# liyi14/mx-DeepIM

Hardware: NVIDIA H100
Metric: 480x640 4-iter pose refinements/sec (higher is better)
Workload: dtype fp16

## Files before the change

mx-deepim_b200/csrc/conv_igemm.cuh:

```cuda
#pragma once
#include <cuda.h>
#include <cuda_fp16.h>
#include "common.cuh"
#include "wgmma.cuh"

namespace dim {

struct ConvKParams {
  CUtensorMap a_map[4];
  CUtensorMap a_lo_map[4];
  CUtensorMap b_map;
  CUtensorMap b_lo_map;
  CUtensorMap out_map[2];
  const __nv_bfloat16 *in_hi, *in_lo;
  int in_cols;
  int KH, KW, stride, cchunks;
  int BW, BH, n_col_tiles;
  int Hq, Ho, Wo, Bn;
  int out_Hp, out_Wp, out_py, out_px, Cout;
  int kblocks;
  float slope;
  const float *bias;
  __nv_bfloat16 *out_hi, *out_lo;
  int in_off_r, in_off_c;
// ... 117 lines not shown
  d |= (uint64_t)((lbo_bytes >> 4) & 0x3FFFu) << 16;
  d |= (uint64_t)((sbo_bytes >> 4) & 0x3FFFu) << 32;
  d |= (uint64_t)layout << 62;
  return d;
}
constexpr uint32_t kSW128 = 1u, kSW64 = 2u, kNoSwizzle = 0u;

__device__ __forceinline__ void regs_producer() { asm volatile("setmaxnreg.dec.sync.aligned.u32 40;"); }
__device__ __forceinline__ void regs_consumer() { asm volatile("setmaxnreg.inc.sync.aligned.u32 232;"); }

}

__device__ __forceinline__ uint32_t pack2_f16(float a, float b) {
  uint32_t r;
  asm("cvt.rn.satfinite.f16x2.f32 %0, %1, %2;" : "=r"(r) : "f"(b), "f"(a));
  return r;
}
__device__ __forceinline__ uint32_t pack2_bf16(float a, float b) {
  uint32_t r;
  asm("cvt.rn.bf16x2.f32 %0, %1, %2;" : "=r"(r) : "f"(b), "f"(a));
  return r;
}

constexpr int kConv1Slack = 2048;


__device__ __forceinline__ int frag_row(int t) { return ((t >> 5) << 4) + ((t & 31) >> 2); }

__device__ __forceinline__ uint32_t pack2_bf16_lo(float v0, float v1, uint32_t hi) {
  return pack2_bf16(v0 - __uint_as_float(hi << 16), v1 - __uint_as_float(hi & 0xFFFF0000u));
}

template <bool SPLIT3, bool F16>
__device__ __forceinline__ void epi_pack(float v0, float v1, float b0, float b1, float slope, uint32_t &hi, uint32_t &lo) {
  v0 += b0;
  v1 += b1;
  v0 = v0 > 0.f ? v0 : v0 * slope;
  v1 = v1 > 0.f ? v1 : v1 * slope;
  if (F16) {
    hi = pack2_f16(v0, v1);
  } else {
    hi = pack2_bf16(v0, v1);
    if (SPLIT3) lo = pack2_bf16_lo(v0, v1, hi);
  }
}

template <bool SPLIT3, bool F16>
__device__ __forceinline__ void store_pair(float v0, float v1, float2 b, float slope, __nv_bfloat16 *out_hi, __nv_bfloat16 *out_lo,
                                           long long off) {
  uint32_t h, l = 0;
  epi_pack<SPLIT3, F16>(v0, v1, b.x, b.y, slope, h, l);
  *reinterpret_cast<uint32_t *>(out_hi + off) = h;
  if (SPLIT3) *reinterpret_cast<uint32_t *>(out_lo + off) = l;
}

template <bool SPLIT3>
__device__ __forceinline__ void store_pair_generic(float v0, float v1, const ConvKParams &p, int n, bool valid, long long off,
                                                   long long add_off, long long mask_off) {
  if (!valid || n >= p.Cout) return;
  if (p.bias) {
    v0 += __ldg(p.bias + n);
    v1 += __ldg(p.bias + n + 1);
  }
  if (p.addend.p) {
    const __nv_bfloat162 a = *reinterpret_cast<const __nv_bfloat162 *>(p.addend.p + add_off);
    if (SPLIT3) {
      const __nv_bfloat162 al = *reinterpret_cast<const __nv_bfloat162 *>(p.addend.lo + add_off);
      v0 += __low2float(a) + __low2float(al);
      v1 += __high2float(a) + __high2float(al);
    } else {
      v0 += __low2float(a);
      v1 += __high2float(a);
    }
  }
  if (p.mask.p) {
    if (n < p.mask_climit) {
      const __nv_bfloat162 m = *reinterpret_cast<const __nv_bfloat162 *>(p.mask.p + mask_off);
      if (!(__low2float(m) > 0.f)) v0 *= p.slope;
      if (!(__high2float(m) > 0.f)) v1 *= p.slope;
    }
  } else {
    v0 = v0 > 0.f ? v0 : v0 * p.slope;
    v1 = v1 > 0.f ? v1 : v1 * p.slope;
  }
  if (SPLIT3) {
    const uint32_t h = pack2_bf16(v0, v1);
    *reinterpret_cast<uint32_t *>(p.out_hi + off) = h;
    *reinterpret_cast<uint32_t *>(p.out_lo + off) = pack2_bf16_lo(v0, v1, h);
  } else {
    *reinterpret_cast<__nv_bfloat162 *>(p.out_hi + off) = __floats2bfloat162_rn(v0, v1);
  }
}

template <int BLOCK_N, int STAGES, bool SPLIT3, int EPI>
struct ConvSmem2 {
  static constexpr int A_BYTES = 128 * 64 * 2;
  static constexpr int B_BYTES = BLOCK_N * 64 * 2;
  static constexpr int NPREC = SPLIT3 ? 2 : 1;
  static constexpr int STAGE_BYTES = (A_BYTES + B_BYTES) * NPREC;
  static constexpr int RING_BYTES = STAGES * STAGE_BYTES;
  static constexpr int LIMIT = 227 * 1024, FIXED = 1024  + 256 ;
  static constexpr bool TMA_EPI = EPI == 0 && !SPLIT3;
  static constexpr int STG_GROUPS =
      !TMA_EPI ? 0 : (RING_BYTES + 2 * BLOCK_N * 128 + FIXED <= LIMIT ? BLOCK_N / 64 : BLOCK_N / 128);
  static constexpr int STG_ROUNDS = TMA_EPI ? BLOCK_N / 64 / STG_GROUPS : 0;
  static constexpr int STG_BYTES = STG_GROUPS * 8192;
// ... 230 lines not shown
  const int g_lo = ck * rows_per_chunk;
  const int g_hi = min(rows_total, g_lo + rows_per_chunk);
  const int n_rows = max(0, g_hi - g_lo);
  const int n_strips = n_rows > 0 ? n_rows + 3 : 0;
  const int ow0 = ct * N;

  if (threadIdx.x == 0) {
    for (int s = 0; s < STAGES; ++s) {
      ptx::mbar_init(&full_bar[s], 1);
      ptx::mbar_init(&empty_bar[s], 2);
    }
    ptx::mbar_init(res_bar, 1);
    ptx::fence_barrier_init();
    ptx::prefetch_tmap(&p.b_map);
    ptx::prefetch_tmap(&p.out_map[0]);
  }
  __syncthreads();

  if (wgi == 0) {
    ptx::regs_producer();
    if (warp == 0 && n_rows > 0) {
      if (ptx::elect_one()) {
        ptx::mbar_expect_tx_raw(res_bar, (uint32_t)S::RES_BYTES);
        for (int kb = 0; kb < 16; ++kb) {
          ptx::tma_load_2d_raw(res + kb * S::TAP_BYTES, &p.b_map, res_bar, kb * 32, 0);
          if (SPLIT3) ptx::tma_load_2d_raw(res + (16 + kb) * S::TAP_BYTES, &p.b_lo_map, res_bar, kb * 32, 0);
        }
      }
      __syncwarp();
      const size_t plane = (size_t)p.in_cols * 16;
      const uint8_t *src_hi = reinterpret_cast<const uint8_t *>(p.in_hi) + (size_t)ow0 * 16;
      const uint8_t *src_lo = reinterpret_cast<const uint8_t *>(p.in_lo) + (size_t)ow0 * 16;
      for (int s = 0; s < n_strips; ++s) {
        const int slot = s % STAGES;
        ptx::mbar_wait(&empty_bar[slot], (((uint32_t)(s / STAGES)) & 1u) ^ 1u);
        uint8_t *st = ring + slot * S::STAGE_BYTES;
        if (g_lo + s >= rows_total) {
          if (ptx::elect_one()) ptx::mbar_arrive(&full_bar[slot]);
        } else if (ptx::elect_one()) {
          ptx::mbar_expect_tx_raw(&full_bar[slot], (uint32_t)(4 * S::PLANE_BYTES * S::NPREC));
          const size_t row = (size_t)(g_lo + s) * 4 * plane;
#pragma unroll
          for (int c = 0; c < 4; ++c) {
            ptx::bulk_load_raw(st + c * S::PLANE_BYTES, src_hi + row + c * plane, S::PLANE_BYTES, &full_bar[slot]);
            if (SPLIT3)
              ptx::bulk_load_raw(st + S::STRIP_BYTES + c * S::PLANE_BYTES, src_lo + row + c * plane, S::PLANE_BYTES, &full_bar[slot]);
          }
        }
        __syncwarp();
      }
    }
  } else if (n_rows > 0) {
    ptx::regs_consumer();
    const int set = wgi - 1, t = threadIdx.x & 127, lane = t & 31;
    const bool leader = t == 0;
    const int co = frag_row(t);
    const float b0 = __ldg(p.bias + co), b1 = __ldg(p.bias + co + 8);
    const uint32_t ring_a = ptx::smem_u32(ring);
    const uint64_t dring = ptx::gmma_desc(ring_a, S::PLANE_BYTES, 128, ptx::kNoSwizzle);
    const uint64_t dring3 = ptx::gmma_desc(ring_a, 2u * S::PLANE_BYTES, 128, ptx::kNoSwizzle) + 3u;
    const uint64_t lo_step = (uint64_t)(S::STRIP_BYTES >> 4);
    const uint64_t slot_step = (uint64_t)(S::STAGE_BYTES >> 4);
    const uint64_t kstep = (uint64_t)(2 * S::PLANE_BYTES >> 4);
    const uint64_t dres = ptx::gmma_desc(ptx::smem_u32(res), 16, 512, ptx::kSW64);
    const uint64_t dres_lo = dres + (uint64_t)((16 * S::TAP_BYTES) >> 4);
    uint8_t *my_stg = stg + set * S::NPREC * S::STG_BYTES;
    const int st_px = ((lane >> 4) << 3) + (lane & 7), st_chunk = 2 * (t >> 5) + ((lane >> 3) & 1);
    const uint32_t st_addr = ptx::smem_u32(my_stg) + (uint32_t)(st_px * 128 + ((st_chunk ^ (lane & 7)) << 4));
    ptx::mbar_wait(res_bar, 0);
    if (set == 1 && leader) ptx::mbar_arrive(&empty_bar[0]);
    for (int row = set; row < n_rows; row += 2) {
      float acc[N / 2];
#pragma unroll
      for (int dh = 0; dh < 4; ++dh) {
        const int s = row + dh;
        ptx::mbar_wait(&full_bar[s % STAGES], ((uint32_t)(s / STAGES)) & 1u);
      }
      wg::fence_acc(acc);
      wg::fence();
#pragma unroll
      for (int dh = 0; dh < 4; ++dh) {
        const uint64_t so = (uint64_t)((row + dh) % STAGES) * slot_step;
#pragma unroll
        for (int k = 0; k < 2; ++k) {
#pragma unroll
          for (int dw = 0; dw < 4; ++dw) {
            if ((dh == 3 || dw == 3) && k == 1) continue;
            const uint64_t db = (dw == 3 ? dring3 : dring + (uint64_t)dw + (uint64_t)k * kstep) + so;
            const uint64_t wo = (uint64_t)((dh * 4 + dw) * (S::TAP_BYTES >> 4) + 2 * k);
            wg::mma<N, F16, 0, 0>(acc, dres + wo, db, (dh | dw | k) ? 1u : 0u);
            if (SPLIT3) {
              wg::mma<N, false, 0, 0>(acc, dres + wo, db + lo_step, 1u);
              wg::mma<N, false, 0, 0>(acc, dres_lo + wo, db, 1u);
            }
          }
        }
      }
      wg::commit();
      wg::wait<0>();
      wg::fence_acc(acc);
      if (leader) {
        ptx::mbar_arrive(&empty_bar[row % STAGES]);
        ptx::mbar_arrive(&empty_bar[(row + 1) % STAGES]);
      }
      const int g = g_lo + row;
      const int n_img = g / p.Hq, oh = g - n_img * p.Hq;
      if (n_img < p.Bn && oh < p.Ho) {
        if (leader) ptx::bulk_wait_read0();
        ptx::named_bar_sync(1 + set, 128);
#pragma unroll
        for (int i = 0; i < N / 16; ++i) {
          uint32_t h[4], l[4] = {0, 0, 0, 0};
          epi_pack<SPLIT3, F16>(acc[8 * i + 0], acc[8 * i + 1], b0, b0, p.slope, h[0], l[0]);
          epi_pack<SPLIT3, F16>(acc[8 * i + 2], acc[8 * i + 3], b1, b1, p.slope, h[1], l[1]);
          epi_pack<SPLIT3, F16>(acc[8 * i + 4], acc[8 * i + 5], b0, b0, p.slope, h[2], l[2]);
          epi_pack<SPLIT3, F16>(acc[8 * i + 6], acc[8 * i + 7], b1, b1, p.slope, h[3], l[3]);
          ptx::stmatrix_x4_trans(st_addr + (uint32_t)(i * 16 * 128), h);
          if (SPLIT3) ptx::stmatrix_x4_trans(st_addr + (uint32_t)(S::STG_BYTES + i * 16 * 128), l);
        }
        ptx::fence_proxy_async();
        ptx::named_bar_sync(1 + set, 128);
        if (leader) {
#pragma unroll
          for (int q = 0; q < N / kConv1StoreN; ++q) {
            ptx::tma_store_4d(&p.out_map[0], my_stg + q * kConv1StoreN * 128, 0, ow0 + q * kConv1StoreN, oh, n_img);
            if (SPLIT3)
              ptx::tma_store_4d(&p.out_map[1], my_stg + S::STG_BYTES + q * kConv1StoreN * 128, 0, ow0 + q * kConv1StoreN, oh, n_img);
          }
          ptx::bulk_commit();
        }
      }
    }
    if (leader) ptx::bulk_wait0();
  }
}

template <int STAGES, bool SPLIT3, bool F16, int NB>
__global__ void __launch_bounds__(384, 1) conv1_rgbd_kernel(const __grid_constant__ ConvKParams p, const int rows_total,
                                                            const int rows_per_chunk, const int chunks_per_col,
                                                            const int strip_bytes ) {
  constexpr int NPREC = SPLIT3 ? 2 : 1;
  constexpr int TAP_BYTES = NB * 128, RES_BYTES = 16 * TAP_BYTES * NPREC;
  extern __shared__ uint8_t smem_raw[];
  uint8_t *smem = reinterpret_cast<uint8_t *>((reinterpret_cast<uintptr_t>(smem_raw) + 1023) & ~(uintptr_t)1023);
  uint8_t *res = smem;
  uint8_t *ring = smem + RES_BYTES;
  const int stage_bytes = strip_bytes * NPREC;
  uint64_t *full_bar = reinterpret_cast<uint64_t *>(ring + STAGES * stage_bytes + kConv1Slack);
  uint64_t *empty_bar = full_bar + STAGES;
  uint64_t *res_bar = empty_bar + STAGES;

  const int wgi = threadIdx.x >> 7, warp = threadIdx.x >> 5;
  const int R = p.BW + 3;
  const uint32_t LBO = (uint32_t)R * 16u;
  const int per_split = p.n_col_tiles * chunks_per_col;
  const int nsplit = blockIdx.x / per_split, cidx = blockIdx.x - nsplit * per_split;
  const int ct = cidx / chunks_per_col, ck = cidx - ct * chunks_per_col;
  const int n0 = nsplit * NB;
  const int g_lo = ck * rows_per_chunk;
  const int g_hi = min(rows_total, g_lo + rows_per_chunk);
  const int n_rows = max(0, g_hi - g_lo);
  const int n_strips = n_rows > 0 ? n_rows + 3 : 0;
  const int ow0 = ct * p.BW;

  if (threadIdx.x == 0) {
    for (int s = 0; s < STAGES; ++s) {
      ptx::mbar_init(&full_bar[s], 1);
      ptx::mbar_init(&empty_bar[s], 2);
    }
    ptx::mbar_init(res_bar, 1);
    ptx::fence_barrier_init();
    ptx::prefetch_tmap(&p.b_map);
    ptx::prefetch_tmap(&p.a_map[0]);
  }
  __syncthreads();

  if (wgi == 0) {
    ptx::regs_producer();
    if (warp == 0 && n_rows > 0) {
      if (ptx::elect_one()) {
// ... 99 lines not shown
```

mx-deepim_b200/csrc/net.cu:

```cuda
#include <cuda_fp16.h>
#include <string.h>

#include <memory>
#include <mutex>

#include "launch.cuh"
#include "net_state.cuh"

namespace dim {

static void build_geometry(NetState *ns, int H, int W) {
  int h = H, w = W;
  for (int i = 0; i < 10; ++i) {
    const LayerSpec &s = kLayers[i];
    LayerGeom &g = ns->g[i];
    g.Cin = s.Cin; g.Cout = s.Cout; g.k = s.k; g.stride = s.stride; g.pad = s.pad;
    g.Hin = h; g.Win = w;
    g.Ho = (h + 2 * s.pad - s.k) / s.stride + 1;
    g.Wo = (w + 2 * s.pad - s.k) / s.stride + 1;
    if (g.Ho < 1) g.Ho = 1;
    if (g.Wo < 1) g.Wo = 1;
    int Hp = h + 2 * s.pad, Wp = w + 2 * s.pad;
    if (s.stride == 2) { Hp += Hp & 1; Wp += Wp & 1; }
    g.py = g.px = s.pad;
    if (i == 0 && ns->input_depth) {
      g.Cin = 10;
      g.rows = Hp / 2; g.cols = Wp / 2; g.Cbuf = 64;
      g.KH = g.KW = 4; g.stride_eff = 1; g.Ceff = 64; g.Hq = g.rows;
      g.BLOCK_K = 64; g.BLOCK_N = 64;
    } else if (i == 0) {
      g.rows = Hp / 2; g.cols = Wp / 2; g.Cbuf = 32;
      g.KH = g.KW = 4; g.stride_eff = 1; g.Ceff = 32; g.Hq = g.rows;
      g.BLOCK_K = 32; g.BLOCK_N = 64;
    } else {
      g.rows = Hp; g.cols = Wp; g.Cbuf = s.Cin;
      g.KH = g.KW = s.k; g.stride_eff = s.stride; g.Ceff = s.Cin;
      g.Hq = (s.stride == 2) ? Hp / 2 : Hp;
      g.BLOCK_K = 64; g.BLOCK_N = s.Cout >= 256 ? 256 : 128;
    }
    int best_bw = 0, best_score = -1;
    for (int pass = 0; pass < 2 && best_bw == 0; ++pass)
      for (int d = 1; d <= g.Wo && d <= 128; ++d) {
        if (g.Wo % d) continue;
        if (pass == 0 && d < 8) continue;
        const int score = d * (128 / d) * 1000 + d;
        if (score > best_score) { best_score = score; best_bw = d; }
      }
    if (best_bw == 0) best_bw = 1;
    g.BW = best_bw; g.BH = 128 / best_bw;
    g.n_col_tiles = g.Wo > 0 ? g.Wo / g.BW : 0;
    if (i == 0) {
      const int nt = cdiv(g.Wo, 128);
      g.BW = cdiv(g.Wo, nt); g.BH = 1; g.n_col_tiles = nt;
    }
    g.kblocks = g.KH * g.KW * (g.Ceff / g.BLOCK_K);
    h = g.Ho; w = g.Wo;
  }
}

typedef CUresult (*EncodeTiledFn)(CUtensorMap *, CUtensorMapDataType, cuuint32_t, void *, const cuuint64_t *,
                                  const cuuint64_t *, const cuuint32_t *, const cuuint32_t *, CUtensorMapInterleave,
                                  CUtensorMapSwizzle, CUtensorMapL2promotion, CUtensorMapFloatOOBfill);
static EncodeTiledFn get_encode() {
  static EncodeTiledFn fn = nullptr;
  if (!fn) {
    void *p = nullptr;
    cudaDriverEntryPointQueryResult q;
    if (cudaGetDriverEntryPoint("cuTensorMapEncodeTiled", &p, cudaEnableDefault, &q) == cudaSuccess &&
        q == cudaDriverEntryPointSuccess)
      fn = reinterpret_cast<EncodeTiledFn>(p);
  }
  return fn;
}

int encode_map(CUtensorMap *m, void *base, int rank, const uint64_t *dims, const uint64_t *strides_bytes,
                      const uint32_t *box, int block_k ) {
  EncodeTiledFn fn = get_encode();
  DIM_REQUIRE(fn != nullptr, "cuTensorMapEncodeTiled entry point not available (driver too old?)");
  cuuint64_t gd[5]; cuuint64_t gs[5]; cuuint32_t bx[5]; cuuint32_t es[5];
  for (int i = 0; i < rank; ++i) { gd[i] = dims[i]; bx[i] = box[i]; es[i] = 1; }
  for (int i = 0; i < rank - 1; ++i) gs[i] = strides_bytes[i];
  CUresult r = fn(m, CU_TENSOR_MAP_DATA_TYPE_BFLOAT16, (cuuint32_t)rank, base, gd, gs, bx, es,
                  CU_TENSOR_MAP_INTERLEAVE_NONE,
                  block_k == 64 ? CU_TENSOR_MAP_SWIZZLE_128B
                                : (block_k == 32 ? CU_TENSOR_MAP_SWIZZLE_64B : CU_TENSOR_MAP_SWIZZLE_NONE),
                  CU_TENSOR_MAP_L2_PROMOTION_L2_256B, CU_TENSOR_MAP_FLOAT_OOB_FILL_NONE);
  if (r != CUDA_SUCCESS) {
    set_error("cuTensorMapEncodeTiled failed with CUresult %d (rank %d dims %llu %llu %llu box %u %u %u)", (int)r, rank,
              (unsigned long long)dims[0], (unsigned long long)dims[1], (unsigned long long)(rank > 2 ? dims[2] : 0),
              box[0], box[1], rank > 2 ? box[2] : 0);
    return 3;
  }
  return 0;
}

static int build_maps(NetState *ns, int B, bool f16, TensorMaps &tm) {
  for (int i = 0; i < 10; ++i) {
    const LayerGeom &g = ns->g[i];
    ConvKParams &kp = tm.kp[i];
    memset(&kp, 0, sizeof(kp));
    for (int lo = 0; lo < 2; ++lo) {
      __nv_bfloat16 *base = lo ? ns->act_lo[i] : ns->act_hi[i];
      CUtensorMap *maps = lo ? kp.a_lo_map : kp.a_map;
      const uint32_t box[3] = {(uint32_t)g.BLOCK_K, (uint32_t)g.BW, (uint32_t)(g.BH / 2)};
      if (i == 0 && ns->input_depth) {
        const uint64_t dims[4] = {8, (uint64_t)g.cols, 8, (uint64_t)B * g.rows};
        const uint64_t str[3] = {16, (uint64_t)g.cols * 16, (uint64_t)g.cols * 128};
        const uint32_t box4[4] = {8, (uint32_t)(g.BW + 3), 8, 1};
        if (int rc = encode_map(&maps[0], base, 4, dims, str, box4, 0)) return rc;
        maps[1] = maps[2] = maps[3] = maps[0];
      } else if (i == 0) {
      } else if (g.stride_eff == 1) {
        const uint64_t dims[3] = {(uint64_t)g.Cbuf, (uint64_t)g.cols, (uint64_t)B * g.rows};
        const uint64_t str[2] = {(uint64_t)g.Cbuf * 2, (uint64_t)g.cols * g.Cbuf * 2};
        if (int rc = encode_map(&maps[0], base, 3, dims, str, box, g.BLOCK_K)) return rc;
        maps[1] = maps[2] = maps[3] = maps[0];
      } else {
        for (int ph = 0; ph < 2; ++ph)
          for (int pw = 0; pw < 2; ++pw) {
            const uint64_t dims[3] = {(uint64_t)g.Cbuf, (uint64_t)g.cols / 2, (uint64_t)B * g.rows / 2};
            const uint64_t str[2] = {(uint64_t)2 * g.Cbuf * 2, (uint64_t)2 * g.cols * g.Cbuf * 2};
            __nv_bfloat16 *vb = base + ((size_t)ph * g.cols + pw) * g.Cbuf;
            if (int rc = encode_map(&maps[(ph << 1) | pw], vb, 3, dims, str, box, g.BLOCK_K)) return rc;
          }
      }
    }
    {
      const uint64_t Ktot = (uint64_t)g.KH * g.KW * g.Ceff;
      const uint64_t dims[2] = {Ktot, (uint64_t)g.Cout};
      const uint64_t str[1] = {Ktot * 2};
      const uint32_t box[2] = {(uint32_t)g.BLOCK_K, (uint32_t)(i == 0 && ns->input_depth ? 16 : g.BLOCK_N)};
      __nv_bfloat16 *wop = f16 ? ns->w_f16[i] : ns->w_hi[i];
      if (int rc = encode_map(&kp.b_map, wop, 2, dims, str, box, g.BLOCK_K)) return rc;
      if (int rc = encode_map(&kp.b_lo_map, ns->w_lo[i], 2, dims, str, box, g.BLOCK_K)) return rc;
    }
    kp.KH = g.KH; kp.KW = g.KW; kp.stride = g.stride_eff; kp.cchunks = g.Ceff / g.BLOCK_K;
    kp.BW = g.BW; kp.BH = g.BH; kp.n_col_tiles = g.n_col_tiles;
    kp.Hq = g.Hq; kp.Ho = g.Ho; kp.Wo = g.Wo; kp.Bn = B;
    if (i < 9) {
      const LayerGeom &nx = ns->g[i + 1];
      kp.out_Hp = nx.rows; kp.out_Wp = nx.cols; kp.out_py = nx.py; kp.out_px = nx.px;
    } else {
      kp.out_Hp = g.Ho; kp.out_Wp = g.Wo; kp.out_py = 0; kp.out_px = 0;
    }
    kp.Cout = g.Cout;
    kp.kblocks = g.kblocks;
    kp.slope = 0.1f;
    kp.bias = ns->bias[i];
    kp.out_hi = ns->act_hi[i + 1];
    kp.out_lo = ns->act_lo[i + 1];
    if (i == 0 && !ns->input_depth) {
      kp.in_hi = ns->act_hi[0];
      kp.in_lo = ns->act_lo[0];
      kp.in_cols = g.cols;
    }
    if (i > 0 || !ns->input_depth) {
      DIM_REQUIRE(i == 0 || (g.BH % 2 == 0 && g.BH / 2 <= g.Hq && g.BW * (g.BH / 2) <= 64),
                  "conv_igemm: a consumer warpgroup's box must be whole output rows within two images");
      const uint64_t cb = (uint64_t)g.Cout * 2;
      const uint64_t dims[4] = {(uint64_t)g.Cout, (uint64_t)g.Wo, (uint64_t)g.Ho, (uint64_t)B};
      const uint64_t str[3] = {cb, (uint64_t)kp.out_Wp * cb, (uint64_t)kp.out_Hp * kp.out_Wp * cb};
      const uint32_t box[4] = {64, (uint32_t)(i == 0 ? kConv1StoreN : g.BW), (uint32_t)(i == 0 ? 1 : g.BH / 2), 1};
      const size_t interior = ((size_t)kp.out_py * kp.out_Wp + kp.out_px) * g.Cout;
      for (int lo = 0; lo < (i == 0 ? 2 : 1); ++lo)
        if (int rc = encode_map(&kp.out_map[lo], (lo ? ns->act_lo[i + 1] : ns->act_hi[i + 1]) + interior, 4, dims, str, box, 64))
          return rc;
    }
  }
  return 0;
}

template <bool F16>
__device__ __forceinline__ void mma_bf16_16816(float *c, const uint32_t *a, uint32_t b0, uint32_t b1) {
  if (F16)
    asm volatile(
        "mma.sync.aligned.m16n8k16.row.col.f32.f16.f16.f32 {%0,%1,%2,%3}, {%4,%5,%6,%7}, {%8,%9}, {%0,%1,%2,%3};"
        : "+f"(c[0]), "+f"(c[1]), "+f"(c[2]), "+f"(c[3])
        : "r"(a[0]), "r"(a[1]), "r"(a[2]), "r"(a[3]), "r"(b0), "r"(b1));
  else
    asm volatile(
        "mma.sync.aligned.m16n8k16.row.col.f32.bf16.bf16.f32 {%0,%1,%2,%3}, {%4,%5,%6,%7}, {%8,%9}, {%0,%1,%2,%3};"
        : "+f"(c[0]), "+f"(c[1]), "+f"(c[2]), "+f"(c[3])
        : "r"(a[0]), "r"(a[1]), "r"(a[2]), "r"(a[3]), "r"(b0), "r"(b1));
}

template <bool S3, bool F16 = false>
__global__ void __launch_bounds__(256) fc6_mma_kernel(const __nv_bfloat16 *__restrict__ act_hi,
                                                      const __nv_bfloat16 *__restrict__ act_lo,
                                                      const __nv_bfloat16 *__restrict__ w_hi,
                                                      const __nv_bfloat16 *__restrict__ w_lo, int B, int max_batch,
                                                      float *__restrict__ partial) {
  constexpr int PITCH = FC6_KC * 2 + 64;
  __shared__ __align__(16) uint8_t a_hi_s[16 * PITCH];
  __shared__ __align__(16) uint8_t a_lo_s[S3 ? 16 * PITCH : 16];
  const int s = blockIdx.x, k0 = s * FC6_KC;
  const int warp = threadIdx.x >> 5, lane = threadIdx.x & 31, g = lane >> 2, q = lane & 3;
  for (int b0 = 0; b0 < B; b0 += 16) {
    const int nb = min(16, B - b0);
    __syncthreads();
    for (int idx = threadIdx.x; idx < 16 * (FC6_KC / 8); idx += blockDim.x) {
      const int r = idx / (FC6_KC / 8), c8 = idx - r * (FC6_KC / 8);
      uint4 vh = make_uint4(0, 0, 0, 0), vl = make_uint4(0, 0, 0, 0);
      if (r < nb) {
        const size_t o = (size_t)(b0 + r) * FC6_K + k0 + c8 * 8;
        vh = *reinterpret_cast<const uint4 *>(act_hi + o);
        if (S3) vl = *reinterpret_cast<const uint4 *>(act_lo + o);
      }
      *reinterpret_cast<uint4 *>(a_hi_s + r * PITCH + c8 * 16) = vh;
      if (S3) *reinterpret_cast<uint4 *>(a_lo_s + r * PITCH + c8 * 16) = vl;
    }
    __syncthreads();
    float acc[4][4];
#pragma unroll
    for (int t = 0; t < 4; ++t)
#pragma unroll
      for (int e = 0; e < 4; ++e) acc[t][e] = 0.f;
#pragma unroll 2
// ... 222 lines not shown
  if (ns->loaded) DIM_CHECK(cudaDeviceSynchronize());
  if (int rc = net_alloc_weights(ctx)) return rc;
  size_t n[12], off[13] = {0};
  for (int i = 0; i < 10; ++i) {
    const LayerGeom &g = ns->g[i];
    const int cin = i == 0 && !ns->input_depth ? (ns->input_mask ? 8 : 6) : g.Cin;
    n[i] = (size_t)g.Cout * cin * g.k * g.k;
  }
  n[10] = (size_t)256 * FC6_K;
  n[11] = 256 * 256;
  for (int i = 0; i < 12; ++i) off[i + 1] = off[i] + n[i];
  float *stage_p = nullptr;
  DIM_CHECK(cudaMalloc(&stage_p, off[12] * sizeof(float)));
  std::unique_ptr<float, cudaError_t (*)(void *)> stage(stage_p, cudaFree);
  auto put = [](float *dst, const float *src, size_t count) {
    return cudaMemcpy(dst, src, count * sizeof(float), cudaMemcpyHostToDevice);
  };
  const float *w[12];
  for (int i = 0; i < 12; ++i) {
    w[i] = stage.get() + off[i];
    if (i != 10) DIM_CHECK(put(stage.get() + off[i], W[i], n[i]));
  }
  {
    std::vector<float> p((size_t)256 * FC6_K);
    for (int o = 0; o < 256; ++o)
      for (int c = 0; c < 1024; ++c)
        for (int hw = 0; hw < 80; ++hw) p[(size_t)o * FC6_K + (size_t)hw * 1024 + c] = W[10][(size_t)o * FC6_K + (size_t)c * 80 + hw];
    DIM_CHECK(put(stage.get() + off[10], p.data(), n[10]));
  }
  for (int i = 0; i < 10; ++i) DIM_CHECK(put(ns->bias[i], Bv[i], ns->g[i].Cout));
  DIM_CHECK(put(ns->fc6_b, Bv[10], 256));
  DIM_CHECK(put(ns->fc7_b, Bv[11], 256));
  DIM_CHECK(put(ns->rot_w, W[12], 4 * 256));
  DIM_CHECK(put(ns->rot_b, Bv[12], 4));
  DIM_CHECK(put(ns->trans_w, W[13], 3 * 256));
  DIM_CHECK(put(ns->trans_b, Bv[13], 3));
  if (int rc = net_pack_weights(ctx, w, 0, PACK_HI | PACK_LO | PACK_F16)) return rc;
  DIM_CHECK(cudaStreamSynchronize(0));
  ns->loaded = true;
  return 0;
}

template <int BN, int ST, bool S3, bool F16>
static int launch_conv(const ConvKParams &kp, int total_tiles, int n_tiles, int cap, cudaStream_t st) {
  using S = ConvSmem2<BN, ST, S3, 0>;
  static bool attr_set = false;
  if (!attr_set) {
    DIM_CHECK(cudaFuncSetAttribute(conv_igemm_persistent_kernel<BN, ST, S3, F16>, cudaFuncAttributeMaxDynamicSharedMemorySize,
                                   S::TOTAL));
    attr_set = true;
  }
  const int grid = total_tiles < cap ? total_tiles : cap;
  conv_igemm_persistent_kernel<BN, ST, S3, F16><<<grid, 384, S::TOTAL, st>>>(kp, total_tiles, n_tiles);
  DIM_LAUNCH_CHECK();
  return 0;
}

template <int N, int ST, bool S3, bool F16>
static int launch_conv1(const ConvKParams &kp, int grid, int rows_total, int rpc, int chunks, cudaStream_t st) {
  using S = Conv1Smem<N, ST, S3>;
  static bool set = false;
  if (!set) {
    DIM_CHECK(cudaFuncSetAttribute(conv1_kernel<N, ST, S3, F16>, cudaFuncAttributeMaxDynamicSharedMemorySize, S::TOTAL));
    set = true;
  }
  conv1_kernel<N, ST, S3, F16><<<grid, 384, S::TOTAL, st>>>(kp, rows_total, rpc, chunks);
  DIM_LAUNCH_CHECK();
  return 0;
}

template <int ST, bool S3, bool F16, int NB>
static int launch_conv1_rgbd(const ConvKParams &kp, int grid, int rows_total, int rpc, int chunks, int strip_bytes,
                             cudaStream_t st) {
  const int smem_bytes = 16 * NB * 128 * (S3 ? 2 : 1) + ST * (S3 ? 2 : 1) * strip_bytes + kConv1Slack + 1024 + 256;
  DIM_REQUIRE(smem_bytes <= 227 * 1024, "conv1 (RGB-D): image too wide for the rolling-strip ring");
  static int set = 0;
  if (set < smem_bytes) {
    DIM_CHECK(cudaFuncSetAttribute(conv1_rgbd_kernel<ST, S3, F16, NB>, cudaFuncAttributeMaxDynamicSharedMemorySize,
                                   smem_bytes));
    set = smem_bytes;
  }
  conv1_rgbd_kernel<ST, S3, F16, NB><<<grid, 384, smem_bytes, st>>>(kp, rows_total, rpc, chunks, strip_bytes);
  DIM_LAUNCH_CHECK();
  return 0;
}

int net_set_input_depth(dim_ctx *ctx, bool enable) {
  NetState *ns = ctx->net;
  DIM_REQUIRE(ns != nullptr, "net not created");
  if (ns->input_depth == enable) return 0;
  DIM_REQUIRE(!ns->loaded, "dim_ctx_set_input_depth: call it before dim_net_load (this context's weights are loaded)");
  if (!ns->act0_rgb_hi) { ns->act0_rgb_hi = ns->act_hi[0]; ns->act0_rgb_lo = ns->act_lo[0]; }
  ns->input_depth = enable;
  build_geometry(ns, ctx->H, ctx->W);
  ns->maps.clear();
  const LayerGeom &g = ns->g[0];
  const size_t per = (size_t)g.rows * g.cols * g.Cbuf;
  ns->act_elems_per_image[0] = per;
  if (enable && ns->net_ok && !ns->act0_rgbd_hi) {
    if (int rc = dev_alloc(ctx, &ns->act0_rgbd_hi, per * ctx->max_batch, true)) return rc;
    if (int rc = dev_alloc(ctx, &ns->act0_rgbd_lo, per * ctx->max_batch, true)) return rc;
  }
  ns->act_hi[0] = enable ? ns->act0_rgbd_hi : ns->act0_rgb_hi;
  ns->act_lo[0] = enable ? ns->act0_rgbd_lo : ns->act0_rgb_lo;
  return 0;
}
// ... 23 lines not shown
  DIM_REQUIRE(ns && ns->loaded, "dim_net_load has not been called");
  DIM_REQUIRE(B >= 1 && B <= ctx->max_batch, "batch exceeds max_batch");
  DIM_REQUIRE(precision == DIM_PREC_BF16 || precision == DIM_PREC_BF16X3 || precision == DIM_PREC_FP16,
              "unknown precision (DIM_PREC_BF16 / DIM_PREC_BF16X3 / DIM_PREC_FP16)");
  const bool s3 = precision == DIM_PREC_BF16X3, f16 = precision == DIM_PREC_FP16;
  const int key = B + (f16 ? kF16MapKey : 0);
  auto it = ns->maps.find(key);
  if (it == ns->maps.end()) {
    TensorMaps tm;
    if (int rc = build_maps(ns, B, f16, tm)) return rc;
    it = ns->maps.emplace(key, tm).first;
  }
  const TensorMaps &tm = it->second;
  if (ns->repack_done) DIM_CHECK(cudaStreamWaitEvent(st, ns->repack_done, 0));
  if (s3 && ns->lo_stale)
    if (int rc = train_refresh_lo(ctx, st)) return rc;
  if (f16 && ns->f16_stale)
    if (int rc = train_refresh_f16(ctx, st)) return rc;
  if (ns->layer_events) DIM_CHECK(cudaEventRecord(ns->layer_events[0], st));
  for (int i = 0; i < 10; ++i) {
    const LayerGeom &g = ns->g[i];
    const ConvKParams &kp = tm.kp[i];
    const int n_tiles = g.Cout / g.BLOCK_N;
    const int total_tiles = cdiv(B * g.Hq, g.BH) * g.n_col_tiles * n_tiles;
    const int sms = ctx->num_sms;
    int rc;
    if (i == 0 && ns->input_depth) {
      const int nsplit = s3 ? 4 : 1;
      const int rows_total = B * g.Hq;
      int chunks = sms / (g.n_col_tiles * nsplit);
      if (chunks > cdiv(rows_total, 16)) chunks = cdiv(rows_total, 16);
      if (chunks < 1) chunks = 1;
      const int rpc = cdiv(rows_total, chunks);
      chunks = cdiv(rows_total, rpc);
      const int strip_bytes = cdiv((g.BW + 3) * 128, 128) * 128;
      const int grid = g.n_col_tiles * chunks * nsplit;
      rc = s3 ? launch_conv1_rgbd<5, true, false, 16>(kp, grid, rows_total, rpc, chunks, strip_bytes, st)
              : (f16 ? launch_conv1_rgbd<6, false, true, 64>(kp, grid, rows_total, rpc, chunks, strip_bytes, st)
                     : launch_conv1_rgbd<6, false, false, 64>(kp, grid, rows_total, rpc, chunks, strip_bytes, st));
    } else if (i == 0) {
      DIM_REQUIRE(g.Wo == 320 && g.cols >= g.Wo + 3 && g.Hq == g.rows && g.Hq == g.Ho + 3,
                  "conv1_kernel is built for a 480x640 input (320 output columns)");
      const int n_col = g.Wo / (s3 ? 80 : 160);
      const int rows_total = B * g.Hq;
      int chunks = sms / n_col;
      if (chunks > cdiv(rows_total, 16)) chunks = cdiv(rows_total, 16);
      if (chunks < 1) chunks = 1;
      const int rpc = cdiv(rows_total, chunks);
      chunks = cdiv(rows_total, rpc);
      const int grid = n_col * chunks;
      rc = s3 ? launch_conv1<80, 5, true, false>(kp, grid, rows_total, rpc, chunks, st)
              : (f16 ? launch_conv1<160, 8, false, true>(kp, grid, rows_total, rpc, chunks, st)
                     : launch_conv1<160, 8, false, false>(kp, grid, rows_total, rpc, chunks, st));
    } else if (g.BLOCK_N == 128) {
      rc = s3 ? launch_conv<128, 3, true, false>(kp, total_tiles, n_tiles, sms, st)
              : (f16 ? launch_conv<128, 6, false, true>(kp, total_tiles, n_tiles, sms, st)
                     : launch_conv<128, 6, false, false>(kp, total_tiles, n_tiles, sms, st));
    } else {
      rc = s3 ? launch_conv<256, 2, true, false>(kp, total_tiles, n_tiles, sms, st)
              : (f16 ? launch_conv<256, 4, false, true>(kp, total_tiles, n_tiles, sms, st)
                     : launch_conv<256, 4, false, false>(kp, total_tiles, n_tiles, sms, st));
    }
    if (rc) return rc;
    if (ns->layer_events && i < 9) DIM_CHECK(cudaEventRecord(ns->layer_events[i + 1], st));
  }
  if (ns->layer_events) DIM_CHECK(cudaEventRecord(ns->layer_events[10], st));
  if (after_conv) DIM_CHECK(cudaEventRecord(after_conv, st));
  if (s3)
    fc6_mma_kernel<true><<<FC6_SPLITS, 256, 0, st>>>(ns->act_hi[10], ns->act_lo[10], ns->fc6_w_hi, ns->fc6_w_lo, B,
                                                     ctx->max_batch, ns->fc6_partial);
  else if (f16)
    fc6_mma_kernel<false, true><<<FC6_SPLITS, 256, 0, st>>>(ns->act_hi[10], nullptr, ns->fc6_w_f16, nullptr, B,
                                                            ctx->max_batch, ns->fc6_partial);
  else
    fc6_mma_kernel<false><<<FC6_SPLITS, 256, 0, st>>>(ns->act_hi[10], nullptr, ns->fc6_w_hi, nullptr, B,
                                                      ctx->max_batch, ns->fc6_partial);
  DIM_LAUNCH_CHECK();
  head_kernel<<<B, 1024, 0, st>>>(ns->fc6_partial, ctx->max_batch, ns->fc6_b, ns->fc7_wT, ns->fc7_b, ns->rot_w,
                                 ns->rot_b, ns->trans_w, ns->trans_b, zoom_factor, rot_out, trans_out, se3_out, ns->save_h6,
                                 ns->save_h7);
  DIM_LAUNCH_CHECK();
  return 0;
}

bool net_graph_safe(dim_ctx *ctx) {
  NetState *ns = ctx->net;
  return ns && ns->loaded && !ns->layer_events && !ns->train_aliased;
}

int net_layer_profile(dim_ctx *ctx, int enable, float *ms10) {
  NetState *ns = ctx->net;
  DIM_REQUIRE(ns != nullptr, "net not created");
  if (enable && !ns->layer_events) {
    ns->layer_events = new cudaEvent_t[11];
    for (int i = 0; i < 11; ++i) DIM_CHECK(cudaEventCreate(&ns->layer_events[i]));
  }
  if (ms10 && ns->layer_events) {
    DIM_CHECK(cudaDeviceSynchronize());
    for (int i = 0; i < 10; ++i) DIM_CHECK(cudaEventElapsedTime(&ms10[i], ns->layer_events[i], ns->layer_events[i + 1]));
  }
  if (!enable && ns->layer_events) {
    for (int i = 0; i < 11; ++i) cudaEventDestroy(ns->layer_events[i]);
    delete[] ns->layer_events;
    ns->layer_events = nullptr;
  }
  return 0;
// ... 25 lines not shown
```

mx-deepim_b200/csrc/net_state.cuh:

```cuda
#pragma once
#include <map>

#include "conv_igemm.cuh"

namespace dim {

struct LayerSpec {
  const char *name;
  int Cout, Cin, k, stride, pad;
};
static const LayerSpec kLayers[10] = {
    {"flow_conv1", 64, 8, 7, 2, 3},  {"conv2", 128, 64, 5, 2, 2},   {"conv3", 256, 128, 5, 2, 2},
    {"conv3_1", 256, 256, 3, 1, 1},  {"conv4", 512, 256, 3, 2, 1},  {"conv4_1", 512, 512, 3, 1, 1},
    {"conv5", 512, 512, 3, 2, 1},    {"conv5_1", 512, 512, 3, 1, 1}, {"conv6", 1024, 512, 3, 2, 1},
    {"conv6_1", 1024, 1024, 3, 1, 1}};

struct LayerGeom {
  int Cin, Cout, k, stride, pad, Hin, Win, Ho, Wo;
  int rows, cols, Cbuf, py, px;
  int KH, KW, stride_eff, Ceff, Hq;
  int BLOCK_N, BLOCK_K, BW, BH, n_col_tiles, kblocks;
};

struct TensorMaps {
  ConvKParams kp[10];
};

__host__ __device__ inline int conv1_kslot(int dw, int ph, int pw) { return dw == 3 ? pw * 16 + ph * 8 : ph * 16 + pw * 8; }

__device__ __forceinline__ void store_split(__nv_bfloat16 *hi, __nv_bfloat16 *lo, size_t i, float v,
                                            __nv_bfloat16 *f16 = nullptr) {
  const __nv_bfloat16 h = __float2bfloat16_rn(v);
  if (hi) hi[i] = h;
  if (lo) lo[i] = __float2bfloat16_rn(v - __bfloat162float(h));
  if (f16) reinterpret_cast<__half *>(f16)[i] = __float2half_rn(v);
}

struct NetState {
  LayerGeom g[10];
  __nv_bfloat16 *w_hi[10] = {}, *w_lo[10] = {};
  __nv_bfloat16 *w_f16[10] = {};
  float *bias[10] = {};
  __nv_bfloat16 *act_hi[11] = {}, *act_lo[11] = {};
  size_t act_elems_per_image[11] = {};
  __nv_bfloat16 *fc6_w_hi = nullptr, *fc6_w_lo = nullptr;
  __nv_bfloat16 *fc6_w_f16 = nullptr;
  bool train_aliased = false;
  bool f16_stale = false;
  float *fc6_b = nullptr, *fc7_wT = nullptr, *fc7_b = nullptr, *rot_w = nullptr, *rot_b = nullptr,
        *trans_w = nullptr, *trans_b = nullptr;
  float *fc6_partial = nullptr;
  cudaEvent_t *layer_events = nullptr;
  bool loaded = false, net_ok = false;
  bool input_depth = false;
  __nv_bfloat16 *act0_rgb_hi = nullptr, *act0_rgb_lo = nullptr, *act0_rgbd_hi = nullptr, *act0_rgbd_lo = nullptr;
  bool input_mask = true;
  float *save_h6 = nullptr, *save_h7 = nullptr;
  cudaEvent_t repack_done = nullptr;
  bool lo_stale = false;
  std::map<int, TensorMaps> maps;
  int max_batch = 0;
};

static constexpr int FC6_K = 1024 * 8 * 10;
static constexpr int FC6_KC = 256;
static constexpr int FC6_SPLITS = FC6_K / FC6_KC;


int encode_map(CUtensorMap *m, void *base, int rank, const uint64_t *dims, const uint64_t *strides_bytes,
               const uint32_t *box, int block_k );
static constexpr int kF16MapKey = 1 << 20;

}
```

Before: 3381.

## Add dedicated tail conv kernel for small late layers with multi-image tiles

Adds a persistent warp-specialized implicit-GEMM kernel for the small late conv layers (output height up to 16, Cout a multiple of 256). Each tile packs several images' whole 8-row output bands into a 160-pixel MMA N dimension, and each consumer warpgroup accumulates CW 64-channel weight strips. The aim is better weight reuse and fuller tiles where the generic kernel's boxes waste lanes on tiny spatial extents. The transposed epilogue staging is pulled into a shared helper. Tile geometry, TMA boxes and out-map encoding change for those layers, which risks mismatches and lower occupancy with a large accumulator.

```diff
diff --git a/mx-deepim_b200/csrc/conv_igemm.cuh b/mx-deepim_b200/csrc/conv_igemm.cuh
--- a/mx-deepim_b200/csrc/conv_igemm.cuh
+++ b/mx-deepim_b200/csrc/conv_igemm.cuh
@@ -193,6 +193,25 @@
   epi_pack<SPLIT3, F16>(v0, v1, b.x, b.y, slope, h, l);
   *reinterpret_cast<uint32_t *>(out_hi + off) = h;
   if (SPLIT3) *reinterpret_cast<uint32_t *>(out_lo + off) = l;
+}
+
+template <int N, bool SPLIT3, bool F16>
+__device__ __forceinline__ void stage_transposed(const float (&acc)[N / 2], float b0, float b1, float slope, uint32_t stg,
+                                                 uint32_t lo_off, int t) {
+  static_assert(N % 16 == 0, "stage_transposed: whole 16-pixel column pairs");
+  const int lane = t & 31;
+  const int st_px = ((lane >> 4) << 3) + (lane & 7), st_chunk = 2 * (t >> 5) + ((lane >> 3) & 1);
+  const uint32_t st_addr = stg + (uint32_t)(st_px * 128 + ((st_chunk ^ (lane & 7)) << 4));
+#pragma unroll
+  for (int i = 0; i < N / 16; ++i) {
+    uint32_t h[4], l[4] = {0, 0, 0, 0};
+    epi_pack<SPLIT3, F16>(acc[8 * i + 0], acc[8 * i + 1], b0, b0, slope, h[0], l[0]);
+    epi_pack<SPLIT3, F16>(acc[8 * i + 2], acc[8 * i + 3], b1, b1, slope, h[1], l[1]);
+    epi_pack<SPLIT3, F16>(acc[8 * i + 4], acc[8 * i + 5], b0, b0, slope, h[2], l[2]);
+    epi_pack<SPLIT3, F16>(acc[8 * i + 6], acc[8 * i + 7], b1, b1, slope, h[3], l[3]);
+    ptx::stmatrix_x4_trans(st_addr + (uint32_t)(i * 16 * 128), h);
+    if (SPLIT3) ptx::stmatrix_x4_trans(st_addr + lo_off + (uint32_t)(i * 16 * 128), l);
+  }
 }
 
 template <bool SPLIT3>
@@ -529,7 +548,7 @@
     }
   } else if (n_rows > 0) {
     ptx::regs_consumer();
-    const int set = wgi - 1, t = threadIdx.x & 127, lane = t & 31;
+    const int set = wgi - 1, t = threadIdx.x & 127;
     const bool leader = t == 0;
     const int co = frag_row(t);
     const float b0 = __ldg(p.bias + co), b1 = __ldg(p.bias + co + 8);
@@ -542,8 +561,6 @@
     const uint64_t dres = ptx::gmma_desc(ptx::smem_u32(res), 16, 512, ptx::kSW64);
     const uint64_t dres_lo = dres + (uint64_t)((16 * S::TAP_BYTES) >> 4);
     uint8_t *my_stg = stg + set * S::NPREC * S::STG_BYTES;
-    const int st_px = ((lane >> 4) << 3) + (lane & 7), st_chunk = 2 * (t >> 5) + ((lane >> 3) & 1);
-    const uint32_t st_addr = ptx::smem_u32(my_stg) + (uint32_t)(st_px * 128 + ((st_chunk ^ (lane & 7)) << 4));
     ptx::mbar_wait(res_bar, 0);
     if (set == 1 && leader) ptx::mbar_arrive(&empty_bar[0]);
     for (int row = set; row < n_rows; row += 2) {
@@ -585,16 +602,7 @@
       if (n_img < p.Bn && oh < p.Ho) {
         if (leader) ptx::bulk_wait_read0();
         ptx::named_bar_sync(1 + set, 128);
-#pragma unroll
-        for (int i = 0; i < N / 16; ++i) {
-          uint32_t h[4], l[4] = {0, 0, 0, 0};
-          epi_pack<SPLIT3, F16>(acc[8 * i + 0], acc[8 * i + 1], b0, b0, p.slope, h[0], l[0]);
-          epi_pack<SPLIT3, F16>(acc[8 * i + 2], acc[8 * i + 3], b1, b1, p.slope, h[1], l[1]);
-          epi_pack<SPLIT3, F16>(acc[8 * i + 4], acc[8 * i + 5], b0, b0, p.slope, h[2], l[2]);
-          epi_pack<SPLIT3, F16>(acc[8 * i + 6], acc[8 * i + 7], b1, b1, p.slope, h[3], l[3]);
-          ptx::stmatrix_x4_trans(st_addr + (uint32_t)(i * 16 * 128), h);
-          if (SPLIT3) ptx::stmatrix_x4_trans(st_addr + (uint32_t)(S::STG_BYTES + i * 16 * 128), l);
-        }
+        stage_transposed<N, SPLIT3, F16>(acc, b0, b1, p.slope, ptx::smem_u32(my_stg), S::STG_BYTES, t);
         ptx::fence_proxy_async();
         ptx::named_bar_sync(1 + set, 128);
         if (leader) {
@@ -603,6 +611,154 @@
             ptx::tma_store_4d(&p.out_map[0], my_stg + q * kConv1StoreN * 128, 0, ow0 + q * kConv1StoreN, oh, n_img);
             if (SPLIT3)
               ptx::tma_store_4d(&p.out_map[1], my_stg + S::STG_BYTES + q * kConv1StoreN * 128, 0, ow0 + q * kConv1StoreN, oh, n_img);
+          }
+          ptx::bulk_commit();
+        }
+      }
+    }
+    if (leader) ptx::bulk_wait0();
+  }
+}
+
+template <int N, int CW, int STAGES, bool SPLIT3>
+struct ConvTailSmem {
+  static constexpr int A_BYTES = CW * 128 * 64 * 2;
+  static constexpr int B_BYTES = N * 64 * 2;
+  static constexpr int NPREC = SPLIT3 ? 2 : 1;
+  static constexpr int STAGE_BYTES = (A_BYTES + B_BYTES) * NPREC;
+  static constexpr int RING_BYTES = STAGES * STAGE_BYTES;
+  static constexpr int STG_BYTES = N * 128;
+  static constexpr int TOTAL = RING_BYTES + 2 * NPREC * STG_BYTES + 1024  + 256 ;
+  static_assert(N % 16 == 0 && B_BYTES % 1024 == 0, "conv tail band width");
+  static_assert(TOTAL <= 227 * 1024, "conv tail shared memory");
+};
+
+template <int N, int CW, int STAGES, bool SPLIT3, bool F16>
+__global__ void __launch_bounds__(384, 1) conv_igemm_tail_kernel(const __grid_constant__ ConvKParams p, const int total_tiles,
+                                                                 const int n_tiles) {
+  using S = ConvTailSmem<N, CW, STAGES, SPLIT3>;
+  constexpr int MT = CW * 128;
+  constexpr uint32_t SBO = 1024u;
+
+  extern __shared__ uint8_t smem_raw[];
+  uint8_t *smem = reinterpret_cast<uint8_t *>((reinterpret_cast<uintptr_t>(smem_raw) + 1023) & ~(uintptr_t)1023);
+  uint8_t *stg = smem + S::RING_BYTES;
+  uint64_t *full_bar = reinterpret_cast<uint64_t *>(stg + 2 * S::NPREC * S::STG_BYTES);
+  uint64_t *empty_bar = full_bar + STAGES;
+
+  const int wgi = threadIdx.x >> 7, warp = threadIdx.x >> 5;
+  const int n_bands = (p.Ho + p.BH - 1) / p.BH, box_px = p.BW * p.BH, imgs = N / box_px;
+  const int box_bytes = box_px * 128;
+
+  if (threadIdx.x == 0) {
+    for (int s = 0; s < STAGES; ++s) {
+      ptx::mbar_init(&full_bar[s], 1);
+      ptx::mbar_init(&empty_bar[s], 2);
+    }
+    ptx::fence_barrier_init();
+    ptx::prefetch_tmap(&p.b_map);
+    ptx::prefetch_tmap(&p.a_map[0]);
+    ptx::prefetch_tmap(&p.out_map[0]);
+  }
+  __syncthreads();
+
+  if (wgi == 0) {
+    ptx::regs_producer();
+    if (warp == 0) {
+      int s = 0;
+      uint32_t ph = 0;
+      for (int tile = blockIdx.x; tile < total_tiles; tile += gridDim.x) {
+        const int ct = tile % n_tiles, mt = tile / n_tiles;
+        const int img = mt / n_bands * imgs, band = mt % n_bands;
+        const int g0 = img * p.Hq + band * p.BH, n0 = ct * MT;
+        for (int kb = 0; kb < p.kblocks; ++kb) {
+          ptx::mbar_wait(&empty_bar[s], ph ^ 1u);
+          const int tap = kb / p.cchunks, cc = kb - tap * p.cchunks;
+          const int kh = tap / p.KW, kw = tap - kh * p.KW;
+          int view = 0, dr = kh, dc = kw;
+          if (p.stride == 2) {
+            view = ((kh & 1) << 1) | (kw & 1);
+            dr = kh >> 1;
+            dc = kw >> 1;
+          }
+          uint8_t *st = smem + s * S::STAGE_BYTES;
+          if (ptx::elect_one()) {
+            ptx::mbar_expect_tx_raw(&full_bar[s], (uint32_t)S::STAGE_BYTES);
+            for (int pr = 0; pr < S::NPREC; ++pr) {
+              uint8_t *sa = st + pr * (S::A_BYTES + S::B_BYTES);
+              for (int c = 0; c < CW; ++c)
+                ptx::tma_load_2d_raw(sa + c * 16384, pr ? &p.b_lo_map : &p.b_map, &full_bar[s], kb * 64, n0 + c * 128);
+              for (int q = 0; q < imgs; ++q)
+                ptx::tma_load_3d_raw(sa + S::A_BYTES + q * box_bytes, pr ? &p.a_lo_map[view] : &p.a_map[view], &full_bar[s],
+                                     cc * 64, dc, g0 + q * p.Hq + dr);
+            }
+          }
+          __syncwarp();
+          if (++s == STAGES) { s = 0; ph ^= 1u; }
+        }
+      }
+    }
+  } else {
+    ptx::regs_consumer();
+    const int t = threadIdx.x & 127;
+    const int half = wgi - 1;
+    const bool leader = t == 0;
+    const uint32_t base = ptx::smem_u32(smem);
+    uint8_t *my_stg = stg + half * S::NPREC * S::STG_BYTES;
+    float acc[CW][N / 2];
+    int s = 0;
+    uint32_t ph = 0;
+    for (int tile = blockIdx.x; tile < total_tiles; tile += gridDim.x) {
+      int prev = -1;
+      for (int kb = 0; kb < p.kblocks; ++kb) {
+        ptx::mbar_wait(&full_bar[s], ph);
+        const uint32_t w_hi = base + s * S::STAGE_BYTES + half * CW * 8192;
+        const uint32_t x_hi = base + s * S::STAGE_BYTES + S::A_BYTES;
+        const uint64_t dw0 = ptx::gmma_desc(w_hi, 16, SBO, ptx::kSW128), dx0 = ptx::gmma_desc(x_hi, 16, SBO, ptx::kSW128);
+        const uint64_t lo = (S::A_BYTES + S::B_BYTES) >> 4;
+#pragma unroll
+        for (int c = 0; c < CW; ++c) wg::fence_acc(acc[c]);
+        wg::fence();
+#pragma unroll
+        for (int k = 0; k < 4; ++k) {
+#pragma unroll
+          for (int c = 0; c < CW; ++c) {
+            const uint64_t dw = dw0 + (uint64_t)(512 * c + 2 * k), dx = dx0 + (uint64_t)(2 * k);
+            wg::mma<N, F16, 0, 0>(acc[c], dw, dx, (kb > 0 || k > 0) ? 1u : 0u);
+            if (SPLIT3) {
+              wg::mma<N, false, 0, 0>(acc[c], dw, dx + lo, 1u);
+              wg::mma<N, false, 0, 0>(acc[c], dw + lo, dx, 1u);
+            }
+          }
+        }
+        wg::commit();
+        wg::wait<1>();
+#pragma unroll
+        for (int c = 0; c < CW; ++c) wg::fence_acc(acc[c]);
+        if (prev >= 0 && leader) ptx::mbar_arrive(&empty_bar[prev]);
+        prev = s;
+        if (++s == STAGES) { s = 0; ph ^= 1u; }
+      }
+      wg::wait<0>();
+#pragma unroll
+      for (int c = 0; c < CW; ++c) wg::fence_acc(acc[c]);
+      if (prev >= 0 && leader) ptx::mbar_arrive(&empty_bar[prev]);
+
+      const int ct = tile % n_tiles, mt = tile / n_tiles;
+      const int img = mt / n_bands * imgs, band = mt % n_bands;
+#pragma unroll
+      for (int c = 0; c < CW; ++c) {
+        const int c0 = ct * MT + (half * CW + c) * 64, co = c0 + frag_row(t);
+        const float b0 = __ldg(p.bias + co), b1 = __ldg(p.bias + co + 8);
+        if (leader) ptx::bulk_wait_read0();
+        ptx::named_bar_sync(1 + half, 128);
+        stage_transposed<N, SPLIT3, F16>(acc[c], b0, b1, p.slope, ptx::smem_u32(my_stg), S::STG_BYTES, t);
+        ptx::fence_proxy_async();
+        ptx::named_bar_sync(1 + half, 128);
+        if (leader) {
+          for (int q = 0; q < imgs && img + q < p.Bn; ++q) {
+            ptx::tma_store_4d(&p.out_map[0], my_stg + q * box_bytes, c0, 0, band * p.BH, img + q);
+            if (SPLIT3) ptx::tma_store_4d(&p.out_map[1], my_stg + S::STG_BYTES + q * box_bytes, c0, 0, band * p.BH, img + q);
           }
           ptx::bulk_commit();
         }
diff --git a/mx-deepim_b200/csrc/net.cu b/mx-deepim_b200/csrc/net.cu
--- a/mx-deepim_b200/csrc/net.cu
+++ b/mx-deepim_b200/csrc/net.cu
@@ -53,6 +53,10 @@
       const int nt = cdiv(g.Wo, 128);
       g.BW = cdiv(g.Wo, nt); g.BH = 1; g.n_col_tiles = nt;
     }
+    g.tail = i > 0 && g.Ho <= 2 * kTailRows && kTailN % (g.Wo * kTailRows) == 0 && g.Cout % 256 == 0;
+    if (g.tail) {
+      g.BW = g.Wo; g.BH = kTailRows; g.n_col_tiles = cdiv(g.Ho, kTailRows); g.BLOCK_N = 128;
+    }
     g.kblocks = g.KH * g.KW * (g.Ceff / g.BLOCK_K);
     h = g.Ho; w = g.Wo;
   }
@@ -102,7 +106,7 @@
     for (int lo = 0; lo < 2; ++lo) {
       __nv_bfloat16 *base = lo ? ns->act_lo[i] : ns->act_hi[i];
       CUtensorMap *maps = lo ? kp.a_lo_map : kp.a_map;
-      const uint32_t box[3] = {(uint32_t)g.BLOCK_K, (uint32_t)g.BW, (uint32_t)(g.BH / 2)};
+      const uint32_t box[3] = {(uint32_t)g.BLOCK_K, (uint32_t)g.BW, (uint32_t)(g.tail ? g.BH : g.BH / 2)};
       if (i == 0 && ns->input_depth) {
         const uint64_t dims[4] = {8, (uint64_t)g.cols, 8, (uint64_t)B * g.rows};
         const uint64_t str[3] = {16, (uint64_t)g.cols * 16, (uint64_t)g.cols * 128};
@@ -155,14 +159,15 @@
       kp.in_cols = g.cols;
     }
     if (i > 0 || !ns->input_depth) {
-      DIM_REQUIRE(i == 0 || (g.BH % 2 == 0 && g.BH / 2 <= g.Hq && g.BW * (g.BH / 2) <= 64),
+      DIM_REQUIRE(i == 0 || g.tail || (g.BH % 2 == 0 && g.BH / 2 <= g.Hq && g.BW * (g.BH / 2) <= 64),
                   "conv_igemm: a consumer warpgroup's box must be whole output rows within two images");
       const uint64_t cb = (uint64_t)g.Cout * 2;
       const uint64_t dims[4] = {(uint64_t)g.Cout, (uint64_t)g.Wo, (uint64_t)g.Ho, (uint64_t)B};
       const uint64_t str[3] = {cb, (uint64_t)kp.out_Wp * cb, (uint64_t)kp.out_Hp * kp.out_Wp * cb};
-      const uint32_t box[4] = {64, (uint32_t)(i == 0 ? kConv1StoreN : g.BW), (uint32_t)(i == 0 ? 1 : g.BH / 2), 1};
+      const uint32_t box[4] = {64, (uint32_t)(i == 0 ? kConv1StoreN : g.BW),
+                               (uint32_t)(i == 0 ? 1 : (g.tail ? g.BH : g.BH / 2)), 1};
       const size_t interior = ((size_t)kp.out_py * kp.out_Wp + kp.out_px) * g.Cout;
-      for (int lo = 0; lo < (i == 0 ? 2 : 1); ++lo)
+      for (int lo = 0; lo < (i == 0 || g.tail ? 2 : 1); ++lo)
         if (int rc = encode_map(&kp.out_map[lo], (lo ? ns->act_lo[i + 1] : ns->act_hi[i + 1]) + interior, 4, dims, str, box, 64))
           return rc;
     }
@@ -491,6 +496,22 @@
   }
   const int grid = total_tiles < cap ? total_tiles : cap;
   conv_igemm_persistent_kernel<BN, ST, S3, F16><<<grid, 384, S::TOTAL, st>>>(kp, total_tiles, n_tiles);
+  DIM_LAUNCH_CHECK();
+  return 0;
+}
+
+template <int N, int CW, int ST, bool S3, bool F16>
+static int launch_conv_tail(const ConvKParams &kp, int groups, int Cout, int cap, cudaStream_t st) {
+  using S = ConvTailSmem<N, CW, ST, S3>;
+  static bool attr_set = false;
+  if (!attr_set) {
+    DIM_CHECK(cudaFuncSetAttribute(conv_igemm_tail_kernel<N, CW, ST, S3, F16>, cudaFuncAttributeMaxDynamicSharedMemorySize,
+                                   S::TOTAL));
+    attr_set = true;
+  }
+  const int n_tiles = Cout / (128 * CW), total_tiles = groups * n_tiles;
+  const int grid = total_tiles < cap ? total_tiles : cap;
+  conv_igemm_tail_kernel<N, CW, ST, S3, F16><<<grid, 384, S::TOTAL, st>>>(kp, total_tiles, n_tiles);
   DIM_LAUNCH_CHECK();
   return 0;
 }
@@ -620,6 +641,11 @@
       rc = s3 ? launch_conv1<80, 5, true, false>(kp, grid, rows_total, rpc, chunks, st)
               : (f16 ? launch_conv1<160, 8, false, true>(kp, grid, rows_total, rpc, chunks, st)
                      : launch_conv1<160, 8, false, false>(kp, grid, rows_total, rpc, chunks, st));
+    } else if (g.tail) {
+      const int groups = cdiv(B, kTailN / (g.BW * g.BH)) * g.n_col_tiles;
+      rc = s3 ? launch_conv_tail<kTailN, 1, 2, true, false>(kp, groups, g.Cout, sms, st)
+              : (f16 ? launch_conv_tail<kTailN, 2, 3, false, true>(kp, groups, g.Cout, sms, st)
+                     : launch_conv_tail<kTailN, 2, 3, false, false>(kp, groups, g.Cout, sms, st));
     } else if (g.BLOCK_N == 128) {
       rc = s3 ? launch_conv<128, 3, true, false>(kp, total_tiles, n_tiles, sms, st)
               : (f16 ? launch_conv<128, 6, false, true>(kp, total_tiles, n_tiles, sms, st)
diff --git a/mx-deepim_b200/csrc/net_state.cuh b/mx-deepim_b200/csrc/net_state.cuh
--- a/mx-deepim_b200/csrc/net_state.cuh
+++ b/mx-deepim_b200/csrc/net_state.cuh
@@ -15,11 +15,14 @@
     {"conv5", 512, 512, 3, 2, 1},    {"conv5_1", 512, 512, 3, 1, 1}, {"conv6", 1024, 512, 3, 2, 1},
     {"conv6_1", 1024, 1024, 3, 1, 1}};
 
+static constexpr int kTailRows = 8, kTailN = 160;
+
 struct LayerGeom {
   int Cin, Cout, k, stride, pad, Hin, Win, Ho, Wo;
   int rows, cols, Cbuf, py, px;
   int KH, KW, stride_eff, Ceff, Hq;
   int BLOCK_N, BLOCK_K, BW, BH, n_col_tiles, kblocks;
+  bool tail;
 };
 
 struct TensorMaps {
```

New measurement: 3444, median of 6. 1.02x the previous value.
